# OxfordML/GPz

Hardware: AMD Instinct MI355X
Metric: objective+gradient evals/sec (higher is better)
Workload: dtype f64

## Files before the change

gpz_amd/csrc/k_moments_ring.hip:

```cpp
#include "gpz_dev.h"
#include "gpz_kernels.h"

#define RG_ROWS 8
#define RG_SLOTS 4
#define RG_JB 2
#define RG_COLS 32
#define RG_SLOT_DOUBLES 640
#define RG_SIDE 512
#define RG_SIDE_RS 96
#define RG_GROUP_REQ 5
#define RG_LDS_BYTES 81920
#define RG_GLDS(g, l) __builtin_amdgcn_global_load_lds((const __attribute__((address_space(1))) void *)(g), (__attribute__((address_space(3))) void *)(l), 16, 0, 0)
static_assert(RG_LDS_BYTES == 4 * RG_SLOTS * RG_SLOT_DOUBLES * 8 && RG_COLS == 16 * RG_JB && RG_SIDE == 2 * RG_ROWS * RG_COLS, "ring size");

template <int D>
__global__ __launch_bounds__(256, 2) void k_moments_ring(RingMomentArgs a) {
    constexpr int NF = 1 + D + D * (D + 1) / 2, XL = D + 2;
    constexpr int NFB = NF >= 64 ? NF / 16 : (NF + 15) / 16;
    constexpr int NL = NF > 16 * NFB ? NF - 16 * NFB : 0;
    static_assert(RG_ROWS * XL <= RG_SIDE_RS, "side block");
    extern __shared__ double rg_smem[];
    const int tid = threadIdx.x, lane = tid & 63, wave = __builtin_amdgcn_readfirstlane(tid >> 6), li = lane & 15, lk = lane >> 4;
    const int ncg = (a.m + 4 * RG_COLS - 1) / (4 * RG_COLS);
    const int cg = blockIdx.x % ncg, chunk = blockIdx.x / ncg;
    const int j0 = cg * (4 * RG_COLS) + wave * RG_COLS;
    if (j0 >= a.m) return;
    double *const ring = rg_smem + wave * (RG_SLOTS * RG_SLOT_DOUBLES);
    const int r_begin = chunk * a.rows_per_chunk;
    const int r_end = min(a.n, r_begin + a.rows_per_chunk);
    const int ng = (r_end - r_begin + RG_ROWS - 1) / RG_ROWS;
    double wj[RG_JB], vj[RG_JB];
#pragma unroll
    for (int cb = 0; cb < RG_JB; ++cb) {
        const int j = min(j0 + 16 * cb + li, a.m - 1);
        wj[cb] = a.w[j];
        vj[cb] = a.v ? a.v[j] : 0.0;
    }
    int fia[NFB], fib[NFB];
#pragma unroll
    for (int fb = 0; fb < NFB; ++fb) {
        const int f = 16 * fb + li;
        int ia = 0, ib = 0;
        if (f >= NF) ia = ib = XL - 1;
        else if (f >= 1) {
            if (f <= D) ia = f;
            else {
                int e2 = f - 1 - D, aa = 0;
                while (e2 >= D - aa) { e2 -= D - aa; ++aa; }
                ia = aa + 1; ib = aa + e2 + 1;
            }
        }
        fia[fb] = ia; fib[fb] = ib;
    }
    int lia[NL > 0 ? NL : 1], lib[NL > 0 ? NL : 1];
#pragma unroll
    for (int t = 0; t < NL; ++t) {
        int e2 = 16 * NFB + t - 1 - D, aa = 0;
        while (e2 >= D - aa) { e2 -= D - aa; ++aa; }
        lia[t] = aa + 1; lib[t] = aa + e2 + 1;
    }
    d4_t acc[RG_JB][NFB];
    double ev[RG_JB][NL + 2];
#pragma unroll
    for (int cb = 0; cb < RG_JB; ++cb) {
#pragma unroll
        for (int fb = 0; fb < NFB; ++fb) acc[cb][fb] = d4_t{0.0, 0.0, 0.0, 0.0};
#pragma unroll
        for (int t = 0; t < NL + 2; ++t) ev[cb][t] = 0.0;
    }
    const unsigned colj = (unsigned)min(j0 + 2 * (lane & 15), a.ld - 2);
    const unsigned voff = (unsigned)(lane >> 4) * (unsigned)a.ld + colj;
    const bool is_rs = lane >= 48;
    const unsigned soff = is_rs ? 2u * (unsigned)(lane - 48) : min(2u * (unsigned)lane, (unsigned)(RG_ROWS * XL - 2));
    const double *const sbase = is_rs ? a.rowscal : a.Xs;
    const unsigned srow = is_rs ? 4u : (unsigned)XL;
    const long last = (long)r_end - 1;
    auto stage_half = [&](int g, int slot, int h) {
        const long rg = (long)r_begin + (long)g * RG_ROWS + 4 * h;
        double *const l0 = ring + slot * RG_SLOT_DOUBLES + 4 * h * RG_COLS;
        if (rg + 4 <= (long)r_end) {
            const size_t ro = (size_t)rg * (size_t)a.ld;
            RG_GLDS(a.Phi + ro + voff, l0);
            RG_GLDS(a.T + ro + voff, l0 + RG_ROWS * RG_COLS);
        } else {
            long row = rg + (lane >> 4);
            row = row < last ? row : last;
            const size_t ro = (size_t)row * (size_t)a.ld + colj;
            RG_GLDS(a.Phi + ro, l0);
            RG_GLDS(a.T + ro, l0 + RG_ROWS * RG_COLS);
        }
    };
    auto stage_side = [&](int g, int slot) {
        const long rg = (long)r_begin + (long)g * RG_ROWS;
        double *const l0 = ring + slot * RG_SLOT_DOUBLES + RG_SIDE;
        long e = rg * (long)srow + (long)soff;
        const long elast = (long)r_end * (long)srow - 2;
        e = e < elast ? e : elast;
        RG_GLDS(sbase + e, l0);
    };
    auto kstep = [&](const double *s0, int kk, int rows_left) {
        const int rr = 4 * kk + lk;
        const bool valid = rr < rows_left;
        const double *xr = s0 + RG_SIDE + rr * XL;
        const double *rs = s0 + RG_SIDE + RG_SIDE_RS + rr * 4;
        const double r0 = rs[0], r1 = rs[1], r2 = rs[2];
        const double ob = valid ? r0 : 0.0, cc = valid ? r1 : 0.0, db = valid ? r2 : 0.0;
        double fr[NFB], fl[NL > 0 ? NL : 1];
#pragma unroll
        for (int fb = 0; fb < NFB; ++fb) fr[fb] = xr[fia[fb]] * xr[fib[fb]];
#pragma unroll
        for (int t = 0; t < NL; ++t) fl[t] = xr[lia[t]] * xr[lib[t]];
        const double *pp = s0 + rr * RG_COLS + li;
        double phn = pp[0], ttn = pp[RG_ROWS * RG_COLS];
        __builtin_amdgcn_sched_barrier(0);
#pragma unroll
        for (int cb = 0; cb < RG_JB; ++cb) {
            const double ph = phn, tt = ttn;
            if (cb + 1 < RG_JB) { phn = pp[16 * (cb + 1)]; ttn = pp[RG_ROWS * RG_COLS + 16 * (cb + 1)]; }
            const double dp = fma(-ob, tt, fma(db, vj[cb], -cc * wj[cb])) * ph;
#pragma unroll
            for (int fb = 0; fb < NFB; ++fb) acc[cb][fb] = MFMA_F64(dp, fr[fb], acc[cb][fb]);
#pragma unroll
            for (int t = 0; t < NL; ++t) ev[cb][t] = fma(dp, fl[t], ev[cb][t]);
            ev[cb][NL] = fma(ph, cc, ev[cb][NL]);
            ev[cb][NL + 1] = fma(ph, db, ev[cb][NL + 1]);
            __builtin_amdgcn_sched_barrier(0);
        }
    };
    for (int g = 0; g < RG_SLOTS; ++g)
        if (g < ng) { stage_half(g, g, 0); stage_half(g, g, 1); stage_side(g, g); }
    for (int g = 0; g < ng; ++g) {
        const int ahead = ng - 1 - g;
        if (ahead >= 3) asm volatile("s_waitcnt vmcnt(15)" ::: "memory");
        else if (ahead == 2) asm volatile("s_waitcnt vmcnt(10)" ::: "memory");
        else if (ahead == 1) asm volatile("s_waitcnt vmcnt(5)" ::: "memory");
        else asm volatile("s_waitcnt vmcnt(0)" ::: "memory");
        const int slot = g % RG_SLOTS;
        const double *s0 = ring + slot * RG_SLOT_DOUBLES;
        const int rows_left = r_end - r_begin - g * RG_ROWS;
        const bool more = g + RG_SLOTS < ng;
        kstep(s0, 0, rows_left);
        asm volatile("s_waitcnt lgkmcnt(0)" ::: "memory");
        if (more) stage_half(g + RG_SLOTS, slot, 0);
        kstep(s0, 1, rows_left);
        asm volatile("s_waitcnt lgkmcnt(0)" ::: "memory");
        if (more) { stage_half(g + RG_SLOTS, slot, 1); stage_side(g + RG_SLOTS, slot); }
    }
    double *rec = a.slab + (size_t)chunk * a.m * (NF + 2);
#pragma unroll
    for (int cb = 0; cb < RG_JB; ++cb) {
#pragma unroll
        for (int r = 0; r < 4; ++r) {
            const int j = j0 + 16 * cb + lk + 4 * r;
            if (j < a.m) {
                double *o = rec + (size_t)j * (NF + 2);
#pragma unroll
                for (int fb = 0; fb < NFB; ++fb)
                    if (16 * fb + li < NF) o[16 * fb + li] = acc[cb][fb][r];
            }
        }
        const int j = j0 + 16 * cb + li;
#pragma unroll
        for (int t = 0; t < NL + 2; ++t) {
            double s = ev[cb][t];
            s += __shfl_xor(s, 16, 64);
            s += __shfl_xor(s, 32, 64);
            if (lk == 0 && j < a.m) rec[(size_t)j * (NF + 2) + (NF - NL) + t] = s;
        }
    }
}

__global__ __launch_bounds__(1024) void k_ring_finish(const double *__restrict__ slab, int nrec, int m, int d, int nf, const double *__restrict__ P,
                                                      const double *__restrict__ xmu, int nm, int mp, double *__restrict__ mom,
                                                      double *__restrict__ cols, int accumulate) {
    __shared__ double part[32][72];
    __shared__ double R[72];
    const int tid = threadIdx.x, j = blockIdx.x, nv = nf + 2;
    const int L = 1024 / nv < 32 ? 1024 / nv : 32;
    const int f = tid % nv, sl = tid / nv;
    if (sl < L) {
        const double *p = slab + (size_t)j * nv + f;
        const size_t stride = (size_t)m * nv;
        double s0 = 0.0, s1 = 0.0, s2 = 0.0, s3 = 0.0;
        int r = sl;
        for (; r + 3 * L < nrec; r += 4 * L) {
            s0 += p[(size_t)r * stride];
            s1 += p[(size_t)(r + L) * stride];
            s2 += p[(size_t)(r + 2 * L) * stride];
            s3 += p[(size_t)(r + 3 * L) * stride];
        }
        for (; r < nrec; r += L) s0 += p[(size_t)r * stride];
        part[sl][f] = (s0 + s1) + (s2 + s3);
    }
    __syncthreads();
    if (tid < nv) {
        double t = 0.0;
        for (int q = 0; q < L; ++q) t += part[q][tid];
        R[tid] = t;
    }
    __syncthreads();
    const int q = tid;
    if (q >= nm + 2) return;
    if (q >= nm) {
        cols[(size_t)(q - nm) * mp + j] = R[nf + (q - nm)];
        return;
    }
    double val;
    if (q < d) {
        const double qc = P[(size_t)j * d + q] - xmu[q];
        val = R[1 + q] - qc * R[0];
    } else {
        int e = q - d, aa = 0;
        while (e >= d - aa) { e -= d - aa; ++aa; }
        const int bb = aa + e;
        const double qa = P[(size_t)j * d + aa] - xmu[aa], qb = P[(size_t)j * d + bb] - xmu[bb];
        val = R[1 + q] - qa * R[1 + bb] - qb * R[1 + aa] + qa * qb * R[0];
    }
    mom[(size_t)j * nm + q] = accumulate ? mom[(size_t)j * nm + q] + val : val;
}

bool moments_ring_fits(int kind, int de, int mp) { return kind == GPZ_KIND_COV && (de == 8 || de == 10) && mp > 256; }
int moments_ring_cols() { return 4 * RG_COLS; }
int moments_ring_features(int de) { return 1 + de + de * (de + 1) / 2; }

template <int D>
static int ring_launch(hipStream_t st, const RingMomentArgs &a, dim3 g) {
    if (hipFuncSetAttribute((const void *)k_moments_ring<D>, hipFuncAttributeMaxDynamicSharedMemorySize, RG_LDS_BYTES) != hipSuccess) return -1;
    hipLaunchKernelGGL(k_moments_ring<D>, g, dim3(256), RG_LDS_BYTES, st, a);
    return hipGetLastError() == hipSuccess ? 0 : -1;
}

int launch_moments_ring(hipStream_t st, const RingMomentArgs &a) {
    if (a.nchunk <= 0) return 0;
    dim3 g((unsigned)((a.m + 4 * RG_COLS - 1) / (4 * RG_COLS)) * (unsigned)a.nchunk);
    switch (a.d) {
        case 8: return ring_launch<8>(st, a, g);
        case 10: return ring_launch<10>(st, a, g);
        default: return -1;
    }
}

void launch_ring_finish(hipStream_t st, const double *slab, int nrec, int m, int d, const double *P, const double *xmu, int nm, int mp,
                        double *mom, double *cols, int accumulate) {
    hipLaunchKernelGGL(k_ring_finish, dim3(m), dim3(1024), 0, st, slab, nrec, m, d, moments_ring_features(d), P, xmu, nm, mp, mom, cols, accumulate);
}
```

Measured before the change: 19.10.

## Specialize steady-state ring loop with compile-time slots and precomputed LDS pointers

Splits the row-group loop into a steady-state phase, unrolled by the four ring slots, and the existing generic tail. In the steady phase, slot offsets and row offsets become compile-time constants. LDS addresses come from hoisted address-space-3 pointers, and global source addresses are advanced incrementally in scalar/vector registers, so no clamping or index arithmetic is needed per step. Leftover-feature index pairs are made constexpr. The aim is to cut address computation and VALU overhead around the MFMA work, at the cost of more code, higher register pressure and hand-written inline asm for carry arithmetic.

```diff
diff --git a/gpz_amd/csrc/k_moments_ring.hip b/gpz_amd/csrc/k_moments_ring.hip
--- a/gpz_amd/csrc/k_moments_ring.hip
+++ b/gpz_amd/csrc/k_moments_ring.hip
@@ -12,6 +12,20 @@
 #define RG_LDS_BYTES 81920
 #define RG_GLDS(g, l) __builtin_amdgcn_global_load_lds((const __attribute__((address_space(1))) void *)(g), (__attribute__((address_space(3))) void *)(l), 16, 0, 0)
 static_assert(RG_LDS_BYTES == 4 * RG_SLOTS * RG_SLOT_DOUBLES * 8 && RG_COLS == 16 * RG_JB && RG_SIDE == 2 * RG_ROWS * RG_COLS, "ring size");
+
+struct RingPair { int ia, ib; };
+constexpr RingPair ring_pair(int D, int f) {
+    int e2 = f - 1 - D, aa = 0;
+    while (e2 >= D - aa) { e2 -= D - aa; ++aa; }
+    return RingPair{aa + 1, aa + e2 + 1};
+}
+template <int D, int F0, int N>
+struct RingLeft {
+    int ia[N > 0 ? N : 1], ib[N > 0 ? N : 1];
+    constexpr RingLeft() : ia{}, ib{} {
+        for (int t = 0; t < N; ++t) { ia[t] = ring_pair(D, F0 + t).ia; ib[t] = ring_pair(D, F0 + t).ib; }
+    }
+};
 
 template <int D>
 __global__ __launch_bounds__(256, 2) void k_moments_ring(RingMomentArgs a) {
@@ -36,6 +50,8 @@
         wj[cb] = a.w[j];
         vj[cb] = a.v ? a.v[j] : 0.0;
     }
+#pragma unroll
+    for (int cb = 0; cb < RG_JB; ++cb) asm volatile("" : "+v"(wj[cb]), "+v"(vj[cb]));
     int fia[NFB], fib[NFB];
 #pragma unroll
     for (int fb = 0; fb < NFB; ++fb) {
@@ -44,21 +60,11 @@
         if (f >= NF) ia = ib = XL - 1;
         else if (f >= 1) {
             if (f <= D) ia = f;
-            else {
-                int e2 = f - 1 - D, aa = 0;
-                while (e2 >= D - aa) { e2 -= D - aa; ++aa; }
-                ia = aa + 1; ib = aa + e2 + 1;
-            }
+            else { ia = ring_pair(D, f).ia; ib = ring_pair(D, f).ib; }
         }
         fia[fb] = ia; fib[fb] = ib;
     }
-    int lia[NL > 0 ? NL : 1], lib[NL > 0 ? NL : 1];
-#pragma unroll
-    for (int t = 0; t < NL; ++t) {
-        int e2 = 16 * NFB + t - 1 - D, aa = 0;
-        while (e2 >= D - aa) { e2 -= D - aa; ++aa; }
-        lia[t] = aa + 1; lib[t] = aa + e2 + 1;
-    }
+    constexpr RingLeft<D, 16 * NFB, NL> left{};
     d4_t acc[RG_JB][NFB];
     double ev[RG_JB][NL + 2];
 #pragma unroll
@@ -98,6 +104,23 @@
         e = e < elast ? e : elast;
         RG_GLDS(sbase + e, l0);
     };
+    auto kmul = [&](double ob, double cc, double db, const double (&fr)[NFB], const double (&fl)[NL > 0 ? NL : 1], auto pp) {
+        double phn = pp(0)[0], ttn = pp(0)[RG_ROWS * RG_COLS];
+        __builtin_amdgcn_sched_barrier(0);
+#pragma unroll
+        for (int cb = 0; cb < RG_JB; ++cb) {
+            const double ph = phn, tt = ttn;
+            if (cb + 1 < RG_JB) { phn = pp(cb + 1)[0]; ttn = pp(cb + 1)[RG_ROWS * RG_COLS]; }
+            const double dp = fma(-ob, tt, fma(db, vj[cb], -cc * wj[cb])) * ph;
+#pragma unroll
+            for (int fb = 0; fb < NFB; ++fb) acc[cb][fb] = MFMA_F64(dp, fr[fb], acc[cb][fb]);
+#pragma unroll
+            for (int t = 0; t < NL; ++t) ev[cb][t] = fma(dp, fl[t], ev[cb][t]);
+            ev[cb][NL] = fma(ph, cc, ev[cb][NL]);
+            ev[cb][NL + 1] = fma(ph, db, ev[cb][NL + 1]);
+            __builtin_amdgcn_sched_barrier(0);
+        }
+    };
     auto kstep = [&](const double *s0, int kk, int rows_left) {
         const int rr = 4 * kk + lk;
         const bool valid = rr < rows_left;
@@ -109,27 +132,82 @@
 #pragma unroll
         for (int fb = 0; fb < NFB; ++fb) fr[fb] = xr[fia[fb]] * xr[fib[fb]];
 #pragma unroll
-        for (int t = 0; t < NL; ++t) fl[t] = xr[lia[t]] * xr[lib[t]];
-        const double *pp = s0 + rr * RG_COLS + li;
-        double phn = pp[0], ttn = pp[RG_ROWS * RG_COLS];
-        __builtin_amdgcn_sched_barrier(0);
-#pragma unroll
-        for (int cb = 0; cb < RG_JB; ++cb) {
-            const double ph = phn, tt = ttn;
-            if (cb + 1 < RG_JB) { phn = pp[16 * (cb + 1)]; ttn = pp[RG_ROWS * RG_COLS + 16 * (cb + 1)]; }
-            const double dp = fma(-ob, tt, fma(db, vj[cb], -cc * wj[cb])) * ph;
-#pragma unroll
-            for (int fb = 0; fb < NFB; ++fb) acc[cb][fb] = MFMA_F64(dp, fr[fb], acc[cb][fb]);
-#pragma unroll
-            for (int t = 0; t < NL; ++t) ev[cb][t] = fma(dp, fl[t], ev[cb][t]);
-            ev[cb][NL] = fma(ph, cc, ev[cb][NL]);
-            ev[cb][NL + 1] = fma(ph, db, ev[cb][NL + 1]);
-            __builtin_amdgcn_sched_barrier(0);
-        }
+        for (int t = 0; t < NL; ++t) fl[t] = xr[left.ia[t]] * xr[left.ib[t]];
+        kmul(ob, cc, db, fr, fl, [&](int cb) { return s0 + rr * RG_COLS + li + 16 * cb; });
     };
     for (int g = 0; g < RG_SLOTS; ++g)
         if (g < ng) { stage_half(g, g, 0); stage_half(g, g, 1); stage_side(g, g); }
-    for (int g = 0; g < ng; ++g) {
+    typedef const __attribute__((address_space(3))) double *lds_t;
+    const int gs = (r_end - r_begin) / RG_ROWS - RG_SLOTS;
+    int g = 0;
+    if (gs > 0) {
+        lds_t xrow = (lds_t)(ring + RG_SIDE + lk * XL), rsp = (lds_t)(ring + RG_SIDE + RG_SIDE_RS + lk * 4);
+        lds_t ppp[RG_JB], xap[NFB], xbp[NFB];
+        asm volatile("" : "+v"(xrow), "+v"(rsp));
+#pragma unroll
+        for (int cb = 0; cb < RG_JB; ++cb) {
+            ppp[cb] = (lds_t)(ring + lk * RG_COLS + li + 16 * cb);
+            asm volatile("" : "+v"(ppp[cb]));
+        }
+#pragma unroll
+        for (int fb = 0; fb < NFB; ++fb) {
+            xap[fb] = xrow + fia[fb];
+            xbp[fb] = xrow + fib[fb];
+            asm volatile("" : "+v"(xap[fb]), "+v"(xbp[fb]));
+        }
+        const size_t hstep = (size_t)4 * (size_t)a.ld * 8;
+        const size_t first = (size_t)(r_begin + RG_SLOTS * RG_ROWS);
+        const char *pP = reinterpret_cast<const char *>(a.Phi + first * (size_t)a.ld);
+        const char *pT = reinterpret_cast<const char *>(a.T + first * (size_t)a.ld);
+        unsigned voffb = voff * 8u;
+        const size_t sp0 = (size_t)(sbase + first * srow + soff);
+        unsigned splo = (unsigned)sp0, sphi = (unsigned)(sp0 >> 32);
+        unsigned sstep = RG_ROWS * 8u * srow;
+        auto kstep_s = [&](auto slotc, auto kkc) {
+            constexpr int so = decltype(slotc)::value * RG_SLOT_DOUBLES, kk = decltype(kkc)::value;
+            const d2_t r01 = *reinterpret_cast<const __attribute__((address_space(3))) d2_t *>(rsp + (so + 16 * kk));
+            const double ob = r01.x, cc = r01.y, db = rsp[so + 16 * kk + 2];
+            double fr[NFB], fl[NL > 0 ? NL : 1];
+#pragma unroll
+            for (int fb = 0; fb < NFB; ++fb) fr[fb] = xap[fb][so + 4 * kk * XL] * xbp[fb][so + 4 * kk * XL];
+#pragma unroll
+            for (int t = 0; t < NL; ++t) fl[t] = xrow[so + 4 * kk * XL + left.ia[t]] * xrow[so + 4 * kk * XL + left.ib[t]];
+            kmul(ob, cc, db, fr, fl, [&](int cb) { return ppp[cb] + (so + 4 * kk * RG_COLS); });
+        };
+        auto request_s = [&](double *l0) {
+            asm volatile("" : "+v"(voffb), "+s"(pP), "+s"(pT));
+            RG_GLDS(pP + voffb, l0);
+            RG_GLDS(pT + voffb, l0 + RG_ROWS * RG_COLS);
+            pP += hstep;
+            pT += hstep;
+        };
+        auto steady = [&](auto slotc) {
+            double *const l0 = ring + decltype(slotc)::value * RG_SLOT_DOUBLES;
+            asm volatile("s_waitcnt vmcnt(15)" ::: "memory");
+            kstep_s(slotc, std::integral_constant<int, 0>{});
+            asm volatile("s_waitcnt lgkmcnt(0)" ::: "memory");
+            request_s(l0);
+            kstep_s(slotc, std::integral_constant<int, 1>{});
+            asm volatile("s_waitcnt lgkmcnt(0)" ::: "memory");
+            request_s(l0 + 4 * RG_COLS);
+            RG_GLDS((const char *)(((size_t)sphi << 32) | splo), l0 + RG_SIDE);
+            const unsigned st = sstep;
+            asm volatile("v_add_co_u32 %0, vcc, %0, %2\n\tv_addc_co_u32 %1, vcc, 0, %1, vcc" : "+v"(splo), "+v"(sphi) : "v"(st) : "vcc");
+        };
+        for (; g + RG_SLOTS <= gs; g += RG_SLOTS) {
+            steady(std::integral_constant<int, 0>{});
+            steady(std::integral_constant<int, 1>{});
+            steady(std::integral_constant<int, 2>{});
+            steady(std::integral_constant<int, 3>{});
+        }
+        if (g < gs) {
+            steady(std::integral_constant<int, 0>{});
+            if (g + 1 < gs) steady(std::integral_constant<int, 1>{});
+            if (g + 2 < gs) steady(std::integral_constant<int, 2>{});
+            g = gs;
+        }
+    }
+    for (; g < ng; ++g) {
         const int ahead = ng - 1 - g;
         if (ahead >= 3) asm volatile("s_waitcnt vmcnt(15)" ::: "memory");
         else if (ahead == 2) asm volatile("s_waitcnt vmcnt(10)" ::: "memory");
```

Measured after the change: 19.21 (median of 6 runs). Within noise of the previous version (+0.6%).
